# JaredWinkens/sdr-iq-visualizer

Hardware: AMD Instinct MI355X
Metric: complex64 IQ Msamples/s through windowed FFT+log-PSD, N=4096; % HBM3E peak (higher is better)
Workload: dtype f32

## Files before the change

### experiments/f4k_order/timeline.py

```python
import argparse
import ctypes
import json
import os
import sys

REPO = os.path.dirname(os.path.dirname(os.path.dirname(os.path.abspath(__file__))))
sys.path.insert(0, REPO)
import torch
import numpy as np
from bench import warm_up_by_time
from sdr_iq_visualizer_amd import _ffi
from sdr_iq_visualizer_amd.spectrum import SpectrumPlan

NFFT = 4096
TICK_NS = 10.0
BIN_MS = 0.5


def analyse(rec, n_frames):
    t = rec[:, 0].astype(np.uint64) | (rec[:, 1].astype(np.uint64) << np.uint64(32))
    assert (t > 0).all(), "frames without a record"
    assert np.array_equal(rec[:, 2], np.arange(n_frames, dtype=np.uint32)), "a record names another frame than its own"
    wg = rec[:, 3].astype(np.int64)
    grid = int(wg.max()) + 1
# ... 8 lines not shown
    cut = np.searchsorted(ms[order], np.arange(n_bins + 1) * BIN_MS, side="left")
    cut[-1] = n_frames
    for b in range(n_bins):
        hi = (b + 1) * BIN_MS
        idx = order[cut[b]:cut[b + 1]]
        if idx.size == 0:
            continue
        reached[wg[idx]] = frame[idx]
        active = (last_ms >= hi) & (reached >= 0)
        front = int(reached.max())
        lag = int(front - reached[active].min()) if active.any() else 0
        bins.append({"ms": round(b * BIN_MS, 2), "frames": int(idx.size), "span": int(frame[idx].max() - frame[idx].min()),
                     "lag_frames": lag, "lag_grids": round(lag / grid, 2)})
    return {"grid": grid, "launch_ms_by_records": round(float(ms.max()), 3), "bins": bins}


def main():
    ap = argparse.ArgumentParser()
    ap.add_argument("--out", required=True)
    ap.add_argument("--frames", type=int, default=1 << 20)
    ap.add_argument("--short", type=int, default=65536)
    ap.add_argument("--pairs", type=int, default=3)
    ap.add_argument("--orders", default="stride,ticket",
                    help="comma-separated SDRK_F4K_ORDER values, each optionally with :<SDRK_F4K_TICKET_FORM> (ticket:rot4)")
    a = ap.parse_args()
    lib = _ffi.lib()
    _ffi.require_device(0)
    set_tl = lib.sdrk_f4k_timeline
    set_tl.argtypes, set_tl.restype = [ctypes.c_void_p], ctypes.c_int
    os.environ["SDRK_F4K_PARTS"] = "1"
    d_in = ctypes.c_void_p()
    _ffi.check(lib.sdrk_dev_alloc(0, a.frames * NFFT * 8, ctypes.byref(d_in)))
    outs = []
    for _ in range(a.pairs):
        p = ctypes.c_void_p()
        _ffi.check(lib.sdrk_dev_alloc(0, a.frames * NFFT * 4, ctypes.byref(p)))
        outs.append(p)
    _ffi.check(lib.sdrk_synth_fill(0, 1234, 0, a.frames, NFFT, d_in, None))
    tl = torch.zeros((a.frames, 4), dtype=torch.int32, device="cuda")
    os.makedirs(os.path.dirname(os.path.abspath(a.out)), exist_ok=True)
    with open(a.out, "a") as out:
        for order in [o for o in a.orders.split(",") if o]:
            os.environ["SDRK_F4K_ORDER"] = order.split(":")[0]
            if ":" in order:
                os.environ["SDRK_F4K_TICKET_FORM"] = order.split(":")[1]
            else:
                os.environ.pop("SDRK_F4K_TICKET_FORM", None)
            with SpectrumPlan(NFFT, window="hann", device=0) as plan:
                warm_up_by_time(lambda: plan.exec_device_timed(d_in.value, a.frames, outs[0].value, 1))
                for i, p in enumerate(outs):
                    for n in (a.frames, a.short):
                        plan.exec_device_timed(d_in.value, n, p.value, 1)
                        tl.zero_()
                        torch.cuda.synchronize()
                        assert set_tl(tl.data_ptr()) == 0
                        ms = plan.exec_device_timed(d_in.value, n, p.value, 1)
                        assert set_tl(None) == 0
                        rec = tl[:n].cpu().numpy().view(np.uint32)
                        r = {"order": order, "pair": i, "frames": n, "launch_ms_by_events": round(float(ms), 4), **analyse(rec, n)}
                        out.write(json.dumps(r) + "\n")
                        out.flush()
                        print(f"== {order} pair {i} frames {n}: {r['launch_ms_by_events']} ms by events, "
                              f"{r['launch_ms_by_records']} ms first to last issue, grid {r['grid']}")
                        for b in r["bins"]:
                            print(f"   {b['ms']:5.2f} ms  frames {b['frames']:7d}  span {b['span']:8d}  lag {b['lag_frames']:8d} "
                                  f"frames = {b['lag_grids']:7.2f} grids", flush=True)
    for p in outs:
        lib.sdrk_dev_free(0, p)
    lib.sdrk_dev_free(0, d_in)

# ... 4 lines not shown
```

### sdr-iq-visualizer_amd/csrc/aux_kernels.hip

```cpp
#include "f4k_deal.h"
#include "kernels.h"
#include "synth_hash.h"

namespace sdrk {

__global__ __launch_bounds__(256) void synth_fill_kernel(uint32_t seed, uint64_t first_frame,
                                                         size_t n_frames, int nfft,
                                                         float4* __restrict__ out) {
    const size_t pairs_per_frame = (size_t)nfft / 2;
    const size_t total = n_frames * pairs_per_frame;
    for (size_t i = (size_t)blockIdx.x * blockDim.x + threadIdx.x; i < total;
         i += (size_t)gridDim.x * blockDim.x) {
        const size_t f = i / pairs_per_frame;
        const uint32_t n = (uint32_t)(i - f * pairs_per_frame) * 2u;
        const uint64_t F = first_frame + f;
        const uint32_t base = synth_frame_base(seed, F);
        int i0, q0, i1, q1;
        synth_codes(base, n, i0, q0);
        synth_codes(base, n + 1u, i1, q1);
        float4 v;
        v.x = (float)i0;
        v.y = (float)q0;
        v.z = (float)i1;
        v.w = (float)q1;
// ... 124 lines not shown
}

hipError_t launch_copy_1to1(const void* d_in, void* d_out, size_t bytes, int num_cus, int blocks_per_cu, hipStream_t stream) {
    const size_t n_vec = bytes / 16;
    if (n_vec == 0) return hipSuccess;
    size_t blocks = (n_vec + 1023) / 1024;
    if (blocks > (size_t)num_cus * blocks_per_cu) blocks = (size_t)num_cus * blocks_per_cu;
    hipLaunchKernelGGL(copy_1to1_kernel, dim3((unsigned)blocks), dim3(256), 0, stream, static_cast<const v4f*>(d_in),
                       static_cast<v4f*>(d_out), n_vec);
    return hipGetLastError();
}

template <class Deal>
__global__ __launch_bounds__(256) void stream_mix_dealt_kernel(const v4f* __restrict__ in, v4f* __restrict__ out, size_t n_frames,
                                                               const sdrk_host::F4kDealArgs da) {
    __shared__ unsigned deal_slot[F4K_DEAL_SLOTS];
    const int tid = threadIdx.x;
    Deal deal = Deal::make(da, n_frames, deal_slot, tid);
    deal.publish(tid);
    __syncthreads();
    deal.begin();
    while (deal.more()) {
        deal.top(tid);
        const size_t f = deal.frame();
        if (f < n_frames) {
            const v4f* x = in + f * 2048;
            v4f* o = out + f * 1024;
            v4f v[8];
#pragma unroll
            for (int j = 0; j < 8; ++j) v[j] = __builtin_nontemporal_load(&x[tid + 256 * j]);
#pragma unroll
            for (int j = 0; j < 4; ++j) __builtin_nontemporal_store(v[2 * j] + v[2 * j + 1], &o[tid + 256 * j]);
        }
        __syncthreads();
        deal.step();
    }
    deal.leave(tid);
}

template <class Deal>
__global__ __launch_bounds__(256) void copy_1to1_dealt_kernel(const v4f* __restrict__ in, v4f* __restrict__ out, size_t n_vec,
                                                              const sdrk_host::F4kDealArgs da) {
    __shared__ unsigned deal_slot[F4K_DEAL_SLOTS];
    const int tid = threadIdx.x;
    const size_t n_units = (n_vec + 1023) / 1024;
    Deal deal = Deal::make(da, n_units, deal_slot, tid);
    deal.publish(tid);
    __syncthreads();
    deal.begin();
    while (deal.more()) {
        deal.top(tid);
        const size_t u = deal.frame();
        if (u < n_units) {
            const size_t i = u * 1024 + tid;
            v4f v[4];
#pragma unroll
            for (int j = 0; j < 4; ++j)
                if (i + 256 * j < n_vec) v[j] = __builtin_nontemporal_load(&in[i + 256 * j]);
#pragma unroll
            for (int j = 0; j < 4; ++j)
                if (i + 256 * j < n_vec) __builtin_nontemporal_store(v[j], &out[i + 256 * j]);
        }
        __syncthreads();
        deal.step();
    }
    deal.leave(tid);
}

template <class Launch>
static hipError_t launch_dealt(sdrk_host::F4kProbeDeal& pd, size_t max_blocks, size_t n_units, Launch&& launch) {
    using namespace sdrk_host;
    if (!pd.d_heads || !f4k_ticket_takes(pd.choice.order, max_blocks, n_units, F4K_TICKET_DEFAULT)) return hipErrorNotSupported;
    const unsigned grid = f4k_ticket_grid(max_blocks, n_units);
    const F4kDealArgs da = {pd.d_heads, pd.bases, pd.choice.form, pd.choice.rot_heads};
    launch(grid, da, pd.choice.rot_heads != 0);
    const hipError_t e = hipGetLastError();
    if (e == hipSuccess && !pd.choice.rot_heads) f4k_ticket_advance(pd.choice.form, pd.bases, n_units, grid);
    return e;
}

hipError_t launch_stream_mix_dealt(const void* d_in, void* d_out, size_t n_frames4096, int num_cus, hipStream_t stream,
                                   sdrk_host::F4kProbeDeal& pd) {
    if (n_frames4096 == 0) return hipSuccess;
    const v4f* in = static_cast<const v4f*>(d_in);
    v4f* out = static_cast<v4f*>(d_out);
    const hipError_t e = launch_dealt(pd, (size_t)num_cus * 3, n_frames4096, [&](unsigned grid, const sdrk_host::F4kDealArgs& da, bool rot) {
        if (rot) hipLaunchKernelGGL(stream_mix_dealt_kernel<F4kRotDeal>, dim3(grid), dim3(256), 0, stream, in, out, n_frames4096, da);
        else hipLaunchKernelGGL(stream_mix_dealt_kernel<F4kTicketDeal>, dim3(grid), dim3(256), 0, stream, in, out, n_frames4096, da);
    });
    return e == hipErrorNotSupported ? launch_stream_mix(d_in, d_out, n_frames4096, num_cus, stream) : e;
}

hipError_t launch_copy_1to1_dealt(const void* d_in, void* d_out, size_t bytes, int num_cus, int blocks_per_cu, hipStream_t stream,
                                  sdrk_host::F4kProbeDeal& pd) {
    const size_t n_vec = bytes / 16;
    if (n_vec == 0) return hipSuccess;
    const v4f* in = static_cast<const v4f*>(d_in);
    v4f* out = static_cast<v4f*>(d_out);
    const hipError_t e = launch_dealt(pd, (size_t)num_cus * blocks_per_cu, (n_vec + 1023) / 1024,
                                      [&](unsigned grid, const sdrk_host::F4kDealArgs& da, bool rot) {
        if (rot) hipLaunchKernelGGL(copy_1to1_dealt_kernel<F4kRotDeal>, dim3(grid), dim3(256), 0, stream, in, out, n_vec, da);
        else hipLaunchKernelGGL(copy_1to1_dealt_kernel<F4kTicketDeal>, dim3(grid), dim3(256), 0, stream, in, out, n_vec, da);
    });
    return e == hipErrorNotSupported ? launch_copy_1to1(d_in, d_out, bytes, num_cus, blocks_per_cu, stream) : e;
}

hipError_t launch_power_mean(const void* d_spec, size_t n_frames, int nfft, float scale, float* d_out,
                             hipStream_t stream) {
    hipLaunchKernelGGL(power_mean_kernel, dim3((nfft + 255) / 256), dim3(256), 0, stream,
                       static_cast<const float2*>(d_spec), n_frames, nfft, scale, d_out);
    return hipGetLastError();
}

}
```

### sdr-iq-visualizer_amd/csrc/f4k_deal.h

```cpp
#pragma once
#include <hip/hip_runtime.h>

#include "f4k_rot.h"
#include "f4k_ticket.h"

namespace sdrk {

constexpr int F4K_DEAL_SLOTS = 4;

__device__ __forceinline__ unsigned f4k_deal_draw(unsigned* word, unsigned n) {
    return __hip_atomic_fetch_add(word, n, __ATOMIC_RELAXED, __HIP_MEMORY_SCOPE_AGENT);
}

struct F4kTicketDeal {
    sdrk_host::F4kTicketForm form;
    size_t n_frames, cur, nx, tn, in_ticket;
    unsigned* head;
    unsigned* slot;
    unsigned hx, base, depth, drawn, par;
    bool last_of_ticket;

    __device__ __forceinline__ F4kTicketDeal(unsigned* heads, const sdrk_host::F4kTicketBases& bases, sdrk_host::F4kTicketForm f,
                                             size_t n, unsigned* lds_slots, int tid)
        : form(f), n_frames(n), in_ticket(f.frames - 1), slot(lds_slots), hx(blockIdx.x & (f.heads - 1)),
          depth(sdrk_host::f4k_ticket_depth(f)), drawn(0), par(1), last_of_ticket(false) {
        head = heads + hx * sdrk_host::F4K_TICKET_HEAD_WORDS + __lane_id();
        base = bases.base[hx];
        if (tid == 0) drawn = f4k_deal_draw(head, depth);
    }
    static __device__ __forceinline__ F4kTicketDeal make(const sdrk_host::F4kDealArgs& a, size_t n, unsigned* lds_slots, int tid) {
        return F4kTicketDeal(a.heads, a.bases, a.form, n, lds_slots, tid);
    }
    __device__ __forceinline__ size_t first_of(unsigned head_value) const {
        return sdrk_host::f4k_ticket_first_frame(form, head_value - base, hx);
    }
    __device__ __forceinline__ void publish(int tid) {
        if (tid == 0) {
// ... 11 lines not shown
    __device__ __forceinline__ void top(int tid) {
        last_of_ticket = ((nx + 1) & in_ticket) == 0;
        if (last_of_ticket && tid == 0) {
            slot[par] = drawn;
            drawn = f4k_deal_draw(head, 1u);
        }
    }
    __device__ __forceinline__ size_t frame() const { return cur; }
    __device__ __forceinline__ size_t next() const { return nx; }
    __device__ __forceinline__ void step() {
        size_t after = nx + 1;
        if (last_of_ticket) {
            after = tn;
            tn = first_of(__builtin_amdgcn_readfirstlane(slot[par]));
            par ^= 1;
        }
        cur = nx;
        nx = after;
    }
    __device__ __forceinline__ void leave(int) {}
};

struct F4kRotDeal {
    sdrk_host::F4kRotDrawer dr;
    size_t n_frames;
    unsigned* lane_heads;
    unsigned* slot;
    unsigned drawn, d0, d1, h0, h1;
    unsigned cur, nx, par;

    __device__ __forceinline__ F4kRotDeal(unsigned* heads, unsigned n_heads, size_t n, unsigned* lds_slots, int tid)
        : dr(sdrk_host::f4k_rot_drawer(n_heads, blockIdx.x)), n_frames(n), lane_heads(heads + __lane_id()), slot(lds_slots),
          drawn(0), d0(0), d1(0), h0(0), h1(0), par(2) {
        if (tid == 0) {
            h0 = dr.head;
            d0 = f4k_deal_draw(word(h0), 1u);
            h1 = (h0 + 1) & (n_heads - 1);
            d1 = f4k_deal_draw(word(h1), 1u);
            dr.head = (h1 + 1) & (n_heads - 1);
            drawn = f4k_deal_draw(word(dr.head), 1u);
            dr.pending = true;
        }
    }
    static __device__ __forceinline__ F4kRotDeal make(const sdrk_host::F4kDealArgs& a, size_t n, unsigned* lds_slots, int tid) {
        return F4kRotDeal(a.heads, a.rot_heads, n, lds_slots, tid);
    }
// ... 18 lines not shown
            slot[par] = dr.pending ? sdrk_host::f4k_rot_take(dr, drawn, n_frames) : sdrk_host::F4K_ROT_NONE;
            if (sdrk_host::f4k_rot_advance(dr)) drawn = f4k_deal_draw(word(dr.head), 1u);
        }
    }
    __device__ __forceinline__ size_t frame() const { return cur; }
    __device__ __forceinline__ size_t next() const { return nx; }
    __device__ __forceinline__ void step() {
        const unsigned after = __builtin_amdgcn_readfirstlane(slot[par]);
        par ^= 1;
        cur = nx;
        nx = after;
    }
    __device__ __forceinline__ void leave(int tid) {
        if (tid == 0) {
            unsigned* const exits = lane_heads + sdrk_host::F4K_ROT_EXIT_WORD;
            if (f4k_deal_draw(exits, 1u) == gridDim.x - 1) {
                for (unsigned x = 0; x < dr.heads; ++x) __hip_atomic_store(word(x), 0u, __ATOMIC_RELAXED, __HIP_MEMORY_SCOPE_AGENT);
                __hip_atomic_store(exits, 0u, __ATOMIC_RELAXED, __HIP_MEMORY_SCOPE_AGENT);
            }
        }
    }
};

}
```

### sdr-iq-visualizer_amd/csrc/f4k_rot.h

```cpp
#pragma once
#include <cstddef>
#include <cstdint>
#include <cstdio>

#include "f4k_ticket.h"

namespace sdrk_host {

constexpr unsigned F4K_ROT_AHEAD = 3;
constexpr unsigned F4K_ROT_EXIT_WORD = F4K_TICKET_MAX_HEADS * F4K_TICKET_HEAD_WORDS;
constexpr unsigned F4K_ROT_WORDS = (F4K_TICKET_MAX_HEADS + 1) * F4K_TICKET_HEAD_WORDS;
constexpr uint32_t F4K_ROT_NONE = 0xFFFFFFFFu;

constexpr bool f4k_rot_heads_ok(unsigned heads) { return heads == 2 || heads == 4 || heads == 8; }

constexpr uint32_t f4k_rot_frame(unsigned heads, uint32_t ticket, unsigned head) { return ticket * heads + head; }

constexpr unsigned f4k_rot_next_head(unsigned heads, unsigned live, unsigned last) {
    const unsigned twice = live | (live << heads);
    return (last + 1 + (unsigned)__builtin_ctz(twice >> (last + 1))) & (heads - 1);
}

struct F4kRotDrawer {
    unsigned heads;
// ... 3 lines not shown
};
constexpr F4kRotDrawer f4k_rot_drawer(unsigned heads, unsigned workgroup) {
    return F4kRotDrawer{heads, (1u << heads) - 1u, workgroup & (heads - 1), false};
}
constexpr uint32_t f4k_rot_take(F4kRotDrawer& d, uint32_t ticket, size_t n_frames) {
    const uint32_t fr = f4k_rot_frame(d.heads, ticket, d.head);
    if (fr >= n_frames) d.live &= ~(1u << d.head);
    return fr;
}
constexpr bool f4k_rot_advance(F4kRotDrawer& d) {
    d.pending = d.live != 0;
    if (d.pending) d.head = f4k_rot_next_head(d.heads, d.live, d.head);
    return d.pending;
}

inline unsigned f4k_rot_parse(const char* s) {
    if (!s || s[0] != 'r' || s[1] != 'o' || s[2] != 't' || s[3] == 0 || s[4] != 0) return 0;
    const unsigned h = (unsigned)(s[3] - '0');
    return f4k_rot_heads_ok(h) ? h : 0;
}

constexpr unsigned F4K_ROT_DEFAULT_HEADS = 4;

struct F4kChoice {
    int order = F4K_ORDER_AUTO;
    F4kTicketForm form = F4K_TICKET_FORM;
    unsigned rot_heads = F4K_ROT_DEFAULT_HEADS;
};
inline F4kChoice f4k_choice(const char* order_env, const char* form_env) {
    F4kChoice c;
    if (order_env) c.order = order_env[0] == 't' ? F4K_ORDER_TICKET : (order_env[0] == 's' ? F4K_ORDER_STRIDE : F4K_ORDER_AUTO);
    if (form_env) {
        F4kTicketForm f = {0, 0};
        if (const unsigned rot = f4k_rot_parse(form_env)) c.rot_heads = rot;
        else if (sscanf(form_env, "%ux%u", &f.heads, &f.frames) == 2 && f4k_ticket_form_ok(f)) { c.form = f; c.rot_heads = 0; }
    }
    return c;
}

struct F4kDealArgs {
    unsigned* heads;
    F4kTicketBases bases;
    F4kTicketForm form;
    unsigned rot_heads;
};

struct F4kProbeDeal {
    F4kChoice choice;
    unsigned* d_heads = nullptr;
    F4kTicketBases bases = {};
};

}
// ... 1 lines not shown
```

### sdr-iq-visualizer_amd/csrc/fft4096.hip

```cpp
#include "f4k_deal.h"
#include "fft4096_core.h"

namespace sdrk {

#ifdef SDRK_F4K_TIMELINE
__device__ uint4* f4k_timeline_buf = nullptr;
#define F4K_TIMELINE_LOAD() uint4* const f4k_tl = f4k_timeline_buf
#define F4K_TIMELINE_MARK(fr)                                                                                   \
    do {                                                                                                        \
        if (f4k_tl && tid == 0 && (fr) < n_frames) {                                                            \
            const unsigned long long f4k_t = wall_clock64();                                                    \
            f4k_tl[fr] = make_uint4((unsigned)f4k_t, (unsigned)(f4k_t >> 32), (unsigned)(fr), blockIdx.x);      \
        }                                                                                                       \
    } while (0)
#else
#define F4K_TIMELINE_LOAD() (void)0
#define F4K_TIMELINE_MARK(fr) (void)0
#endif

template <bool HAS_WINDOW, int EPILOGUE>
__global__ __launch_bounds__(F4K_THREADS, F4K_WAVES) void fft4096_kernel(
    const float2* __restrict__ iq, size_t frame_stride, void* __restrict__ out_raw,
    size_t n_frames, const float* __restrict__ window, const float2* __restrict__ tw4096,
    float eps, int shift) {
// ... 149 lines not shown
        In::issue(x, iq + fr * frame_stride, tid);
    };
    In::word nxt[16];
    deal.begin();
    issue(nxt, deal.frame());
    while (deal.more()) {
        deal.top(tid);
        const size_t cur = deal.frame();
        if (cur < n_frames) {
            In::to_owners(nxt, lds, tid);
            cf v[16];
#pragma unroll
            for (int j = 0; j < 16; ++j) v[j] = In::widen(nxt[j]);
            issue(nxt, deal.next());
            f4k_windowed_transform<HAS_WINDOW>(v, lds, tw256, tw1, lds_win, A, tid);
            deal.step();
            f4k_store_row<EPILOGUE>(v, frame_rsrc(static_cast<char*>(out_raw) + cur * (size_t)(F4K_N * OUT_ELEM), F4K_N * OUT_ELEM),
                                    voff_out, xor_k2, eps);
        } else {
            issue(nxt, deal.next());
            __syncthreads();
            deal.step();
        }
    }
    deal.leave(tid);
}

unsigned f4k_max_blocks(int num_cus) { return f4k_grid(num_cus, F4K_WAVES, (size_t)-1); }

hipError_t launch_fft4096(const LaunchArgs& a) {
    if (a.n_frames == 0) return hipSuccess;
    dim3 g(f4k_grid(a.num_cus, F4K_WAVES, a.n_frames)), b(F4K_THREADS);
    const float2* iq = static_cast<const float2*>(a.d_iq);
    const float2* tw = static_cast<const float2*>(a.d_twiddle);
#define SDRK_LAUNCH(W, E)                                                                            \
    hipLaunchKernelGGL((fft4096_kernel<W, E>), g, b, 0, a.stream, iq, a.frame_stride, a.d_out,           \
                       a.n_frames, a.d_window, tw, a.eps, a.shift)
    if (a.epilogue == EPI_LOGPSD) {
        if (a.d_window) SDRK_LAUNCH(true, EPI_LOGPSD); else SDRK_LAUNCH(false, EPI_LOGPSD);
    } else {
        if (a.d_window) SDRK_LAUNCH(true, EPI_COMPLEX); else SDRK_LAUNCH(false, EPI_COMPLEX);
    }
#undef SDRK_LAUNCH
    return hipGetLastError();
}

// ... 16 lines not shown
    return hipGetLastError();
}

hipError_t launch_fft4096_rot(const LaunchArgs& a, unsigned* d_heads, unsigned n_heads, unsigned grid) {
    if (a.n_frames == 0) return hipSuccess;
    if (!d_heads || grid == 0 || grid % sdrk_host::F4K_TICKET_MAX_HEADS || !sdrk_host::f4k_rot_heads_ok(n_heads) ||
        a.n_frames > sdrk_host::F4K_TICKET_MAX_FRAMES)
        return hipErrorInvalidValue;
    dim3 g(grid), b(F4K_THREADS);
    const float2* iq = static_cast<const float2*>(a.d_iq);
    const float2* tw = static_cast<const float2*>(a.d_twiddle);
#define SDRK_LAUNCH(W, E)                                                                            \
    hipLaunchKernelGGL((fft4096_rot_kernel<W, E>), g, b, 0, a.stream, iq, a.frame_stride, a.d_out,       \
                       a.n_frames, a.d_window, tw, a.eps, a.shift, d_heads, n_heads)
    if (a.epilogue == EPI_LOGPSD) {
        if (a.d_window) SDRK_LAUNCH(true, EPI_LOGPSD); else SDRK_LAUNCH(false, EPI_LOGPSD);
    } else {
        if (a.d_window) SDRK_LAUNCH(true, EPI_COMPLEX); else SDRK_LAUNCH(false, EPI_COMPLEX);
    }
#undef SDRK_LAUNCH
    return hipGetLastError();
}

}

#ifdef SDRK_F4K_TIMELINE
extern "C" int sdrk_f4k_timeline(void* d_records) {
    uint4* p = static_cast<uint4*>(d_records);
    return (int)hipMemcpyToSymbol(HIP_SYMBOL(sdrk::f4k_timeline_buf), &p, sizeof p);
}
#endif
```

### sdr-iq-visualizer_amd/csrc/fft4096_core.h

```cpp
#pragma once
#include "cplx.h"
#include "kernels.h"

namespace sdrk {

constexpr int F4K_N = 4096;
constexpr int F4K_THREADS = 256;
#ifndef F4K_WAVES
#define F4K_WAVES 3
#endif
constexpr int F4K_XCH_ELEMS = 4112;
constexpr int F4K_TW_ELEMS = 512;
#ifndef F4K_NT
#define F4K_NT 2
#endif
constexpr int f4k_lds_elems(bool lds_window) { return F4K_XCH_ELEMS + F4K_TW_ELEMS + (lds_window ? F4K_N / 2 : 0); }

typedef unsigned v2u __attribute__((ext_vector_type(2)));

__device__ __forceinline__ __amdgpu_buffer_rsrc_t frame_rsrc(const void* base, unsigned bytes) {
    return __builtin_amdgcn_make_buffer_rsrc(const_cast<void*>(base), 0, (int)bytes, 0x00020000);
}


// ... 22 lines not shown
    const int lo = tid & 15, hi = tid >> 4;
    tw256[tid] = tw4096[(16 * lo * hi) & (F4K_N - 1)];
    tw1[tid] = tw4096[tid];
}

__device__ __forceinline__ void pow_tree(cf w1, cf (&w)[16]) {
    w[1] = w1;
    w[2] = cmul(w1, w1);
    w[3] = cmul(w[2], w1);
    w[4] = cmul(w[2], w[2]);
    w[5] = cmul(w[4], w1);
    w[6] = cmul(w[4], w[2]);
    w[7] = cmul(w[4], w[3]);
    w[8] = cmul(w[4], w[4]);
    w[9] = cmul(w[8], w1);
    w[10] = cmul(w[8], w[2]);
    w[11] = cmul(w[8], w[3]);
    w[12] = cmul(w[8], w[4]);
    w[13] = cmul(w[8], w[5]);
    w[14] = cmul(w[8], w[6]);
    w[15] = cmul(w[8], w[7]);
}

template <bool WIN = false>
__device__ __forceinline__ void f4k_transform(cf (&v)[16], float2* __restrict__ lds,
                                              const float2* __restrict__ tw256,
                                              const float2* __restrict__ tw1, const F4kAddr& A,
                                              int tid, const float* __restrict__ win = nullptr) {
    radix16<WIN>(v, win);
    {
        const float2 t1 = tw1[tid];
        cf w[16];
        pow_tree(cf{t1.x, t1.y}, w);
#pragma unroll
        for (int k = 1; k < 16; ++k) v[rev16(k)] = cmul(v[rev16(k)], w[k]);
    }
    __syncthreads();
#pragma unroll
    for (int k = 0; k < 16; ++k)
        lds[((k & 1) ? A.x1w_odd : A.x1w_even) + 256 * k] = make_float2(v[rev16(k)].x, v[rev16(k)].y);
    __syncthreads();
#pragma unroll
    for (int j = 0; j < 16; ++j) {
        float2 t = lds[((j & 1) ? A.x1r_odd : A.x1r_even) + 16 * j];
        v[j] = cf{t.x, t.y};
    }
    radix16(v);
#pragma unroll
    for (int k = 1; k < 16; ++k) {
        float2 w = tw256[16 * k + A.lo];
        v[rev16(k)] = cmul(v[rev16(k)], cf{w.x, w.y});
    }
    __syncthreads();
#pragma unroll
    for (int k = 0; k < 16; ++k) lds[A.x2w + 16 * k] = make_float2(v[rev16(k)].x, v[rev16(k)].y);
    __syncthreads();
#pragma unroll
    for (int j = 0; j < 16; ++j) {
        float2 t = lds[tid + 257 * j];
        v[j] = cf{t.x, t.y};
// ... 2 lines not shown
}


inline unsigned f4k_grid(int num_cus, int wg_per_cu, size_t work_items) {
    const size_t max_blocks = (size_t)num_cus * wg_per_cu;
    return (unsigned)(work_items < max_blocks ? work_items : max_blocks);
}

struct F4kInC64 {
    typedef v2u word;
    typedef float2 sample;
    static __device__ __forceinline__ void issue(word (&x)[16], const sample* frame, int tid) {
        __amdgpu_buffer_rsrc_t r = frame_rsrc(frame, F4K_N * 8);
#pragma unroll
        for (int j = 0; j < 16; ++j) x[j] = __builtin_amdgcn_raw_buffer_load_b64(r, tid * 8, j * 2048, F4K_NT);
    }
    static __device__ __forceinline__ void to_owners(word (&)[16], float2*, int) {}
    static __device__ __forceinline__ cf widen(word w) {
        v2f t = __builtin_bit_cast(v2f, w);
        return cf{t.x, t.y};
    }
};

template <bool HAS_WINDOW>
__device__ __forceinline__ void f4k_windowed_transform(cf (&v)[16], float2* __restrict__ lds, const float2* __restrict__ tw256,
                                                       const float2* __restrict__ tw1, const float* __restrict__ lds_win,
                                                       const F4kAddr& A, int tid) {
    if (HAS_WINDOW) {
        float win[16];
#pragma unroll
        for (int j = 0; j < 16; ++j) win[j] = lds_win[tid + 256 * j];
        f4k_transform<true>(v, lds, tw256, tw1, A, tid, win);
    } else {
        f4k_transform(v, lds, tw256, tw1, A, tid);
    }
}

template <int EPILOGUE>
__device__ __forceinline__ void f4k_store_row(const cf (&v)[16], __amdgpu_buffer_rsrc_t w, int voff, int xor_k2, float eps) {
    if (EPILOGUE == EPI_LOGPSD) {
#pragma unroll
        for (int k2 = 0; k2 < 16; ++k2) {
            cf z = v[rev16(k2)];
            float db = logpsd_db(z.x, z.y, eps);
            __builtin_amdgcn_raw_buffer_store_b32(__builtin_bit_cast(unsigned, db), w, voff, (k2 ^ xor_k2) * 1024, F4K_NT);
        }
    } else {
#pragma unroll
        for (int k2 = 0; k2 < 16; ++k2) {
            cf z = v[rev16(k2)];
            v2f o = {z.x, z.y};
            __builtin_amdgcn_raw_buffer_store_b64(__builtin_bit_cast(v2u, o), w, voff, (k2 ^ xor_k2) * 2048, 0);
        }
    }
}

}
// ... 1 lines not shown
```

### sdr-iq-visualizer_amd/csrc/kernels.h

```cpp
#pragma once
#include <hip/hip_runtime.h>
#include <stddef.h>
#include <stdint.h>

#include <atomic>

#include "f4k_ticket.h"
#include "f4k_rot.h"

#ifdef SDRK_PHASE_MARKS
#define SDRK_PHASE(name) asm volatile("; SDRK_PHASE " name ::: "memory")
#else
#define SDRK_PHASE(name) do { } while (0)
#endif

namespace sdrk {

enum Epilogue : int {
    EPI_LOGPSD = 0,
    EPI_COMPLEX = 1,
    EPI_BLU_MUL = 2,
    EPI_BLU_POST_LOG = 3,
    EPI_BLU_POST_C64 = 4,
};
// ... 34 lines not shown
__device__ __forceinline__ float logpsd_db_fast(float p) {
    return __builtin_amdgcn_logf(p) * 3.01029995663981195213f;
}

#endif

inline hipError_t ensure_dynamic_lds(const void* kernel, size_t lds_bytes, std::atomic<uint64_t>& mask) {
    if (lds_bytes <= 64 * 1024) return hipSuccess;
    int dev = 0;
    hipError_t e = hipGetDevice(&dev);
    if (e != hipSuccess) return e;
    const uint64_t bit = (dev >= 0 && dev < 64) ? (uint64_t)1 << dev : 0;
    if (bit && (mask.load(std::memory_order_acquire) & bit)) return hipSuccess;
    e = hipFuncSetAttribute(kernel, hipFuncAttributeMaxDynamicSharedMemorySize, (int)lds_bytes);
    if (e == hipSuccess && bit) mask.fetch_or(bit, std::memory_order_release);
    return e;
}

hipError_t launch_fft4096(const LaunchArgs& a);
unsigned f4k_max_blocks(int num_cus);
hipError_t launch_fft4096_ticket(const LaunchArgs& a, unsigned* d_heads, const sdrk_host::F4kTicketBases& bases,
                                 sdrk_host::F4kTicketForm form, unsigned grid);
hipError_t launch_fft4096_rot(const LaunchArgs& a, unsigned* d_heads, unsigned n_heads, unsigned grid);
hipError_t launch_fft_small(const LaunchArgs& a);
bool fft_lds_supports(int nfft);
hipError_t launch_fft_lds(const LaunchArgs& a);
bool fft_tiled2_split(int nfft, int* log2a, int* log2m);
hipError_t launch_fft_tiled2(const LaunchArgs& a);
bool fft_tiled2_has_mip(int nfft, int epilogue);
hipError_t launch_synth_fill(uint32_t seed, uint64_t first_frame, size_t n_frames, int nfft,
                             void* d_iq, hipStream_t stream);

size_t fused64k_ring_bytes();
size_t fused64k_ctrl_words();
unsigned fused64k_sets(int num_cus);
hipError_t launch_fused64k(const LaunchArgs& a, void* d_ring, unsigned* d_ctrl);
bool blu_fused_supports(int M);
hipError_t launch_blu_fused(const void* d_iq, size_t frame_stride, size_t n_frames, int N, int M, const float* d_window,
                            const void* d_chirp, const void* d_bspec, const void* d_twM, float eps, int shift,
                            int epilogue, void* d_out, int num_cus, hipStream_t s);
hipError_t launch_blu_pre(const void* d_iq, size_t frame_stride, size_t n_frames, int N, int M, const float* d_window,
                          const void* d_chirp, void* d_a, int num_cus, hipStream_t s, bool compact = false);
hipError_t launch_blu_mul(const void* d_A, const void* d_B, size_t n_frames, int M, void* d_out, int num_cus,
                          hipStream_t s);
hipError_t launch_blu_post(const void* d_Y, const void* d_chirp, size_t n_frames, int N, int M, float eps, int shift,
                           int epilogue, void* d_out, int num_cus, hipStream_t s);
// ... 25 lines not shown
```

### sdr-iq-visualizer_amd/csrc/plan_internal.h

```cpp
#pragma once
#include <hip/hip_runtime.h>

#include <cstddef>
#include <cstdint>
#include <map>
#include <mutex>
#include <utility>
#include <vector>

#include "../../include/sdrk.h"
#include "kernels.h"

namespace sdrk_host {
constexpr int HOST_SLOTS = 3;
struct ChunkOut {
    enum Rows {
        None,
        Pooled,
        Direct,
        Kernel,
        Planes,
    } rows = None;
    void* user = nullptr;
    size_t bytes = 0;
// ... 72 lines not shown
    int precision = 32;
    double eps64 = 0.0;
    double* d_window64 = nullptr;
    double* d_tw64 = nullptr;
    void* d_scratch64 = nullptr;
    sdrk_host::Staging ci16;
    sdrk_host::Staging integ;
    float* d_pfb_h = nullptr;
    int pfb_taps = 0;
    int pfb_assign = 0;
    sdrk_host::Staging pfb;
    float2* d_fir_h = nullptr;
    int fir_taps = 0;
    int fir_assign = 0;
    float2* d_beam_h = nullptr;
    int beam_channels = 0;
    int beam_taps = 0;
    int f4k_order = sdrk_host::F4K_ORDER_AUTO;
    sdrk_host::F4kTicketForm f4k_form = sdrk_host::F4K_TICKET_FORM;
    unsigned* d_f4k_heads = nullptr;
    sdrk_host::F4kTicketBases f4k_bases = {};
    unsigned f4k_rot_heads = sdrk_host::F4K_ROT_DEFAULT_HEADS;
    unsigned* d_f4k_rot = nullptr;
    hipEvent_t f4k_ev = nullptr;
    hipStream_t f4k_last = nullptr;
    bool f4k_recorded = false;
    size_t f4k_parts = 0;
};

namespace sdrk_host {

constexpr size_t SMALL_IN_BYTES = 256 << 10;
constexpr size_t HOST_CHUNK_BYTES = 16 << 20;
constexpr size_t ZERO_COPY_MAX_BYTES = 32 << 20;
constexpr unsigned FUSED_MAILBOX = 64;
constexpr size_t FUSED_AUTO_MIN_FRAMES = 512;

int fail(int status, const char* fmt, ...) __attribute__((format(printf, 2, 3)));

#define HIP_TRY(expr)                                                                                                   \
    do {                                                                                                                \
        hipError_t e__ = (expr);                                                                                        \
        if (e__ != hipSuccess)                                                                                          \
            return ::sdrk_host::fail(e__ == hipErrorOutOfMemory ? SDRK_ERR_NOMEM : SDRK_ERR_HIP,                        \
                                     "%s failed: %s (%s:%d)", #expr, hipGetErrorString(e__), __FILE__, __LINE__);       \
    } while (0)
// ... 197 lines not shown
```

### sdr-iq-visualizer_amd/csrc/sdrk_plan.hip

```cpp
#include "../../include/sdrk.h"

#include <hip/hip_runtime.h>

#include <cmath>
#include <cstdio>
#include <cstdlib>
#include <cstring>
#include <dlfcn.h>
#include <mutex>
#include <new>
#include <vector>

#include "f4k_split.h"
#include "kernels.h"
#include "plan_internal.h"

using namespace sdrk_host;

namespace sdrk_host {

struct EpiArgs {
    const float2* tab = nullptr;
    int n_out = 0;
    float eps = 0.0f;
// ... 129 lines not shown
            if (st != SDRK_OK) return st;
            e = sdrk::launch_blu_mul(p->d_blu_b, p->d_blu_bspec, nf, M, p->d_blu_a, p->num_cus, stream);
            if (e != hipSuccess) break;
            st = plan_launch(p->blu_inner, p->d_blu_a, nf, (size_t)M, p->d_blu_b, sdrk::EPI_COMPLEX, stream);
            if (st != SDRK_OK) return st;
            e = sdrk::launch_blu_post(p->d_blu_b, p->d_blu_chirp, nf, N, M, p->eps, p->shift, epilogue,
                                      static_cast<char*>(d_out) + f0 * (size_t)N * out_elem, p->num_cus, stream);
            if (e != hipSuccess) break;
        }
    } else if (p->nfft == 4096) {
        const size_t max_blocks = sdrk::f4k_max_blocks(p->num_cus);
        const bool ticket = p->d_f4k_heads && f4k_ticket_takes(p->f4k_order, max_blocks, n_frames, F4K_TICKET_DEFAULT);
        size_t parts = p->f4k_parts ? p->f4k_parts : (ticket ? f4k_ticket_parts(n_frames) : f4k_split_parts(n_frames));
        if (p->f4k_parts && parts > n_frames) parts = n_frames ? n_frames : 1;
        const size_t per = (n_frames + parts - 1) / parts;
        const size_t out_elem = epilogue == sdrk::EPI_LOGPSD ? sizeof(float) : sizeof(float2);
        if (ticket && p->f4k_recorded && p->f4k_last != stream) e = hipStreamWaitEvent(stream, p->f4k_ev, 0);
        for (size_t f0 = 0; f0 < n_frames && e == hipSuccess; f0 += per) {
            a.d_iq = static_cast<const float2*>(d_iq) + f0 * frame_stride;
            a.d_out = static_cast<char*>(d_out) + f0 * (size_t)4096 * out_elem;
            a.n_frames = n_frames - f0 < per ? n_frames - f0 : per;
            if (ticket) {
                const unsigned grid = f4k_ticket_grid(max_blocks, a.n_frames);
                if (p->f4k_rot_heads) {
                    e = sdrk::launch_fft4096_rot(a, p->d_f4k_rot, p->f4k_rot_heads, grid);
                } else {
                    e = sdrk::launch_fft4096_ticket(a, p->d_f4k_heads, p->f4k_bases, p->f4k_form, grid);
                    if (e == hipSuccess) f4k_ticket_advance(p->f4k_form, p->f4k_bases, a.n_frames, grid);
                }
            } else {
                e = sdrk::launch_fft4096(a);
            }
        }
        if (ticket && e == hipSuccess) {
            e = hipEventRecord(p->f4k_ev, stream);
            p->f4k_last = stream;
            p->f4k_recorded = true;
        }
    } else if (sdrk::fft_lds_supports(p->nfft))
        e = sdrk::launch_fft_lds(a);
    else if (p->nfft < 4096)
        e = sdrk::launch_fft_small(a);
    else if (takes_fused(p, call_frames) && !d_mip && epilogue <= sdrk::EPI_COMPLEX) {
        FusedGate& gate = fused_gate(p->device);
        std::lock_guard<std::mutex> lk(gate.mu);
        if (gate.ev && gate.last_stream != stream && gate.recorded) e = hipStreamWaitEvent(stream, gate.ev, 0);
        if (e == hipSuccess) e = sdrk::launch_fused64k(a, p->d_fused_ring, p->d_fused_ctrl);
// ... 168 lines not shown
            const double ang = M_PI * (double)r / (double)nfft;
            c[n] = make_float2((float)std::cos(ang), (float)std::sin(ang));
            b[n] = c[n];
            if (n) b[M - n] = c[n];
        }
        PLAN_TRY(hipMalloc((void**)&p->d_blu_chirp, sizeof(float2) * nfft));
        PLAN_TRY(hipMemcpy(p->d_blu_chirp, c.data(), sizeof(float2) * nfft, hipMemcpyHostToDevice));
        PLAN_TRY(hipMalloc((void**)&p->d_blu_a, (one_kernel ? 1 : frames) * (size_t)M * sizeof(float2)));
        if (!one_kernel) PLAN_TRY(hipMalloc((void**)&p->d_blu_b, frames * (size_t)M * sizeof(float2)));
        PLAN_TRY(hipMalloc((void**)&p->d_blu_bspec, (size_t)M * sizeof(float2)));
        PLAN_TRY(hipMemcpy(p->d_blu_a, b.data(), sizeof(float2) * M, hipMemcpyHostToDevice));
        st2 = plan_launch(p->blu_inner, p->d_blu_a, 1, (size_t)M, p->d_blu_bspec, sdrk::EPI_COMPLEX, p->stream);
        if (st2 != SDRK_OK) { sdrk_plan_destroy(p); return st2; }
        PLAN_TRY(hipStreamSynchronize(p->stream));
        *out = p;
        return SDRK_OK;
    }
    if (nfft <= 16384) {
        std::vector<float2> t(nfft);
        for (int m = 0; m < nfft; ++m) t[m] = twiddle(m, nfft);
        PLAN_TRY(hipMalloc((void**)&p->d_twiddle, sizeof(float2) * nfft));
        PLAN_TRY(hipMemcpy(p->d_twiddle, t.data(), sizeof(float2) * nfft, hipMemcpyHostToDevice));
        if (nfft == 4096) {
            const F4kChoice choice = f4k_choice(getenv("SDRK_F4K_ORDER"), getenv("SDRK_F4K_TICKET_FORM"));
            p->f4k_order = choice.order;
            p->f4k_form = choice.form;
            p->f4k_rot_heads = choice.rot_heads;
            if (const char* env = getenv("SDRK_F4K_PARTS")) {
                long v = atol(env);
                if (v >= 1 && v <= 4096) p->f4k_parts = (size_t)v;
            }
            PLAN_TRY(hipMalloc((void**)&p->d_f4k_rot, F4K_ROT_WORDS * sizeof(uint32_t)));
            const std::vector<uint32_t> rot0(F4K_ROT_WORDS, 0u);
            PLAN_TRY(hipMemcpy(p->d_f4k_rot, rot0.data(), rot0.size() * sizeof(uint32_t), hipMemcpyHostToDevice));
            std::vector<uint32_t> h(F4K_TICKET_MAX_HEADS * F4K_TICKET_HEAD_WORDS, 0u);
            for (unsigned x = 0; x < F4K_TICKET_MAX_HEADS; ++x) h[x * F4K_TICKET_HEAD_WORDS] = p->f4k_bases.base[x] = 0xFFFFFE00u;
            PLAN_TRY(hipMalloc((void**)&p->d_f4k_heads, h.size() * sizeof(uint32_t)));
            PLAN_TRY(hipMemcpy(p->d_f4k_heads, h.data(), h.size() * sizeof(uint32_t), hipMemcpyHostToDevice));
            PLAN_TRY(hipEventCreateWithFlags(&p->f4k_ev, hipEventDisableTiming));
        }
    } else {
        size_t scratch_mb = 192;
        if (const char* env = getenv("SDRK_SCRATCH_MB")) {
            long v = atol(env);
            if (v >= 1 && v <= 65536) scratch_mb = (size_t)v;
        }
        size_t frames = (scratch_mb << 20) / ((size_t)nfft * sizeof(float2));
        if (frames < 1) frames = 1;
        if (frames > max_batch) frames = max_batch;
        p->scratch_frames = frames;
// ... 164 lines not shown
```

### sdr-iq-visualizer_amd/csrc/sdrk_probes.hip

```cpp
#include "../../include/sdrk.h"

#include <hip/hip_runtime.h>

#include <algorithm>
#include <chrono>
#include <cstring>
#include <vector>

#include "kernels.h"
#include "plan_internal.h"

using namespace sdrk_host;

namespace sdrk_host {
namespace {

thread_local int g_probe_status = SDRK_OK;
hipError_t probe_launch_result(int st) {
    if (st == SDRK_OK) return hipSuccess;
    g_probe_status = st;
    return hipErrorUnknown;
}
int probe_fail(hipError_t e, const char* what) {
    if (e == hipErrorUnknown && g_probe_status != SDRK_OK) {
// ... 60 lines not shown
    hipEvent_t e0 = nullptr, e1 = nullptr;
    HIP_TRY(hipStreamCreateWithFlags(&s, hipStreamNonBlocking));
    hipError_t e = hipEventCreate(&e0);
    if (e == hipSuccess) e = hipEventCreate(&e1);
    for (int i = -2; i < launches && e == hipSuccess; ++i) {
        if (i >= 0) e = hipEventRecord(e0, s);
        if (e == hipSuccess) e = launch(prop.multiProcessorCount, s);
        if (i >= 0 && e == hipSuccess) e = hipEventRecord(e1, s);
        if (i >= 0 && e == hipSuccess) e = hipEventSynchronize(e1);
        if (i >= 0 && e == hipSuccess) e = hipEventElapsedTime(&each_ms[i], e0, e1);
    }
    (void)hipStreamSynchronize(s);
    if (e0) (void)hipEventDestroy(e0);
    if (e1) (void)hipEventDestroy(e1);
    (void)hipStreamDestroy(s);
    if (e != hipSuccess) return fail(SDRK_ERR_HIP, "%s failed: %s", what, hipGetErrorString(e));
    return SDRK_OK;
}

struct ProbeHeads {
    F4kProbeDeal deal;
    int status = SDRK_OK;
    explicit ProbeHeads(int device) {
        deal.choice = f4k_choice(getenv("SDRK_F4K_ORDER"), getenv("SDRK_F4K_TICKET_FORM"));
        if (deal.choice.order == F4K_ORDER_STRIDE) return;
        status = check_device(device);
        if (status != SDRK_OK) return;
        const std::vector<uint32_t> zero(F4K_ROT_WORDS, 0u);
        hipError_t e = hipSetDevice(device);
        if (e == hipSuccess) e = hipMalloc((void**)&deal.d_heads, zero.size() * sizeof(uint32_t));
        if (e == hipSuccess) e = hipMemcpy(deal.d_heads, zero.data(), zero.size() * sizeof(uint32_t), hipMemcpyHostToDevice);
        if (e != hipSuccess) status = fail(SDRK_ERR_HIP, "probe heads: %s", hipGetErrorString(e));
    }
    ~ProbeHeads() {
        if (deal.d_heads) (void)hipFree(deal.d_heads);
    }
    ProbeHeads(const ProbeHeads&) = delete;
    ProbeHeads& operator=(const ProbeHeads&) = delete;
};

}

int tune_staging(sdrk_plan* p) {
    const size_t nfft = (size_t)p->nfft;
    if (p->blu_inner || p->max_batch * nfft * sizeof(float2) <= 2 * HOST_CHUNK_BYTES) return SDRK_OK;
    size_t per = HOST_CHUNK_BYTES / (nfft * sizeof(float2));
    if (per < 1) per = 1;
// ... 313 lines not shown
```

Before: 538,800.

## Add two-ahead rotating-head frame dealer with deferred draw for FFT4096

Adds a new rotating-head work dealer (F4kRotDeal2) that publishes the next frame index at the top of each iteration and issues the atomic draw for the following frame after the compute body. This keeps the atomic's latency off the critical path between frames. A new fft4096_rot2 kernel and dealt copy/mix probe kernels use this dealer, and it becomes the default via SDRK_F4K_ROT_AHEAD. The cost is an extra barrier per iteration, double-buffered LDS slots, and more complex dealing logic.

After: 557,300, median of 6. +3.4%, better.

```diff
diff --git a/experiments/f4k_order/timeline.py b/experiments/f4k_order/timeline.py
--- a/experiments/f4k_order/timeline.py
+++ b/experiments/f4k_order/timeline.py
@@ -54,7 +54,8 @@
     ap.add_argument("--short", type=int, default=65536)
     ap.add_argument("--pairs", type=int, default=3)
     ap.add_argument("--orders", default="stride,ticket",
-                    help="comma-separated SDRK_F4K_ORDER values, each optionally with :<SDRK_F4K_TICKET_FORM> (ticket:rot4)")
+                    help="comma-separated SDRK_F4K_ORDER values, each optionally with :<SDRK_F4K_TICKET_FORM> (ticket:rot4) and, for a "
+                         "rot form, @<SDRK_F4K_ROT_AHEAD> (ticket:rot4@3)")
     a = ap.parse_args()
     lib = _ffi.lib()
     _ffi.require_device(0)
@@ -74,10 +75,12 @@
     with open(a.out, "a") as out:
         for order in [o for o in a.orders.split(",") if o]:
             os.environ["SDRK_F4K_ORDER"] = order.split(":")[0]
-            if ":" in order:
-                os.environ["SDRK_F4K_TICKET_FORM"] = order.split(":")[1]
-            else:
-                os.environ.pop("SDRK_F4K_TICKET_FORM", None)
+            form, _, ahead = order.partition(":")[2].partition("@")
+            for var, value in (("SDRK_F4K_TICKET_FORM", form), ("SDRK_F4K_ROT_AHEAD", ahead)):
+                if value:
+                    os.environ[var] = value
+                else:
+                    os.environ.pop(var, None)
             with SpectrumPlan(NFFT, window="hann", device=0) as plan:
                 warm_up_by_time(lambda: plan.exec_device_timed(d_in.value, a.frames, outs[0].value, 1))
                 for i, p in enumerate(outs):
diff --git a/sdr-iq-visualizer_amd/csrc/aux_kernels.hip b/sdr-iq-visualizer_amd/csrc/aux_kernels.hip
--- a/sdr-iq-visualizer_amd/csrc/aux_kernels.hip
+++ b/sdr-iq-visualizer_amd/csrc/aux_kernels.hip
@@ -170,6 +170,10 @@
     deal.begin();
     while (deal.more()) {
         deal.top(tid);
+        if constexpr (Deal::TWO_AHEAD) {
+            __syncthreads();
+            deal.read();
+        }
         const size_t f = deal.frame();
         if (f < n_frames) {
             const v4f* x = in + f * 2048;
@@ -180,7 +184,8 @@
 #pragma unroll
             for (int j = 0; j < 4; ++j) __builtin_nontemporal_store(v[2 * j] + v[2 * j + 1], &o[tid + 256 * j]);
         }
-        __syncthreads();
+        if constexpr (Deal::TWO_AHEAD) deal.tail(tid);
+        else __syncthreads();
         deal.step();
     }
     deal.leave(tid);
@@ -198,6 +203,10 @@
     deal.begin();
     while (deal.more()) {
         deal.top(tid);
+        if constexpr (Deal::TWO_AHEAD) {
+            __syncthreads();
+            deal.read();
+        }
         const size_t u = deal.frame();
         if (u < n_units) {
             const size_t i = u * 1024 + tid;
@@ -209,7 +218,8 @@
             for (int j = 0; j < 4; ++j)
                 if (i + 256 * j < n_vec) __builtin_nontemporal_store(v[j], &out[i + 256 * j]);
         }
-        __syncthreads();
+        if constexpr (Deal::TWO_AHEAD) deal.tail(tid);
+        else __syncthreads();
         deal.step();
     }
     deal.leave(tid);
@@ -221,7 +231,7 @@
     if (!pd.d_heads || !f4k_ticket_takes(pd.choice.order, max_blocks, n_units, F4K_TICKET_DEFAULT)) return hipErrorNotSupported;
     const unsigned grid = f4k_ticket_grid(max_blocks, n_units);
     const F4kDealArgs da = {pd.d_heads, pd.bases, pd.choice.form, pd.choice.rot_heads};
-    launch(grid, da, pd.choice.rot_heads != 0);
+    launch(grid, da, !pd.choice.rot_heads ? 0 : (pd.choice.rot_ahead == F4K_AHEAD_2TOP ? 2 : 1));
     const hipError_t e = hipGetLastError();
     if (e == hipSuccess && !pd.choice.rot_heads) f4k_ticket_advance(pd.choice.form, pd.bases, n_units, grid);
     return e;
@@ -232,8 +242,9 @@
     if (n_frames4096 == 0) return hipSuccess;
     const v4f* in = static_cast<const v4f*>(d_in);
     v4f* out = static_cast<v4f*>(d_out);
-    const hipError_t e = launch_dealt(pd, (size_t)num_cus * 3, n_frames4096, [&](unsigned grid, const sdrk_host::F4kDealArgs& da, bool rot) {
-        if (rot) hipLaunchKernelGGL(stream_mix_dealt_kernel<F4kRotDeal>, dim3(grid), dim3(256), 0, stream, in, out, n_frames4096, da);
+    const hipError_t e = launch_dealt(pd, (size_t)num_cus * 3, n_frames4096, [&](unsigned grid, const sdrk_host::F4kDealArgs& da, int rot) {
+        if (rot == 2) hipLaunchKernelGGL(stream_mix_dealt_kernel<F4kRotDeal2>, dim3(grid), dim3(256), 0, stream, in, out, n_frames4096, da);
+        else if (rot) hipLaunchKernelGGL(stream_mix_dealt_kernel<F4kRotDeal>, dim3(grid), dim3(256), 0, stream, in, out, n_frames4096, da);
         else hipLaunchKernelGGL(stream_mix_dealt_kernel<F4kTicketDeal>, dim3(grid), dim3(256), 0, stream, in, out, n_frames4096, da);
     });
     return e == hipErrorNotSupported ? launch_stream_mix(d_in, d_out, n_frames4096, num_cus, stream) : e;
@@ -246,8 +257,9 @@
     const v4f* in = static_cast<const v4f*>(d_in);
     v4f* out = static_cast<v4f*>(d_out);
     const hipError_t e = launch_dealt(pd, (size_t)num_cus * blocks_per_cu, (n_vec + 1023) / 1024,
-                                      [&](unsigned grid, const sdrk_host::F4kDealArgs& da, bool rot) {
-        if (rot) hipLaunchKernelGGL(copy_1to1_dealt_kernel<F4kRotDeal>, dim3(grid), dim3(256), 0, stream, in, out, n_vec, da);
+                                      [&](unsigned grid, const sdrk_host::F4kDealArgs& da, int rot) {
+        if (rot == 2) hipLaunchKernelGGL(copy_1to1_dealt_kernel<F4kRotDeal2>, dim3(grid), dim3(256), 0, stream, in, out, n_vec, da);
+        else if (rot) hipLaunchKernelGGL(copy_1to1_dealt_kernel<F4kRotDeal>, dim3(grid), dim3(256), 0, stream, in, out, n_vec, da);
         else hipLaunchKernelGGL(copy_1to1_dealt_kernel<F4kTicketDeal>, dim3(grid), dim3(256), 0, stream, in, out, n_vec, da);
     });
     return e == hipErrorNotSupported ? launch_copy_1to1(d_in, d_out, bytes, num_cus, blocks_per_cu, stream) : e;
diff --git a/sdr-iq-visualizer_amd/csrc/f4k_deal.h b/sdr-iq-visualizer_amd/csrc/f4k_deal.h
--- a/sdr-iq-visualizer_amd/csrc/f4k_deal.h
+++ b/sdr-iq-visualizer_amd/csrc/f4k_deal.h
@@ -13,6 +13,7 @@
 }
 
 struct F4kTicketDeal {
+    static constexpr bool TWO_AHEAD = false;
     sdrk_host::F4kTicketForm form;
     size_t n_frames, cur, nx, tn, in_ticket;
     unsigned* head;
@@ -70,6 +71,7 @@
 };
 
 struct F4kRotDeal {
+    static constexpr bool TWO_AHEAD = false;
     sdrk_host::F4kRotDrawer dr;
     size_t n_frames;
     unsigned* lane_heads;
@@ -134,4 +136,62 @@
     }
 };
 
+struct F4kRotDeal2 {
+    static constexpr bool TWO_AHEAD = true;
+    sdrk_host::F4kRotDrawer dr;
+    size_t n_frames;
+    unsigned* lane_heads;
+    unsigned* slot;
+    unsigned drawn, d0, h0;
+    unsigned cur, nx, par;
+
+    __device__ __forceinline__ F4kRotDeal2(unsigned* heads, unsigned n_heads, size_t n, unsigned* lds_slots, int tid)
+        : dr(sdrk_host::f4k_rot_drawer(n_heads, blockIdx.x)), n_frames(n), lane_heads(heads + __lane_id()), slot(lds_slots),
+          drawn(0), d0(0), h0(0), cur(0), nx(sdrk_host::F4K_ROT_NONE), par(2) {
+        if (tid == 0) {
+            h0 = dr.head;
+            d0 = f4k_deal_draw(word(h0), 1u);
+            dr.head = (h0 + 1) & (n_heads - 1);
+            drawn = f4k_deal_draw(word(dr.head), 1u);
+            dr.pending = true;
+        }
+    }
+    static __device__ __forceinline__ F4kRotDeal2 make(const sdrk_host::F4kDealArgs& a, size_t n, unsigned* lds_slots, int tid) {
+        return F4kRotDeal2(a.heads, a.rot_heads, n, lds_slots, tid);
+    }
+    __device__ __forceinline__ unsigned* word(unsigned head) const { return lane_heads + head * sdrk_host::F4K_TICKET_HEAD_WORDS; }
+    __device__ __forceinline__ void publish(int tid) {
+        if (tid == 0) {
+            const unsigned h1 = dr.head;
+            dr.head = h0;
+            slot[0] = sdrk_host::f4k_rot_take(dr, d0, n_frames);
+            dr.head = h1;
+        }
+    }
+    __device__ __forceinline__ void begin() { cur = __builtin_amdgcn_readfirstlane(slot[0]); }
+    __device__ __forceinline__ bool more() const { return cur != sdrk_host::F4K_ROT_NONE; }
+    __device__ __forceinline__ void top(int tid) {
+        if (tid == 0) slot[par] = dr.pending ? sdrk_host::f4k_rot_take(dr, drawn, n_frames) : sdrk_host::F4K_ROT_NONE;
+    }
+    __device__ __forceinline__ void read() {
+        nx = __builtin_amdgcn_readfirstlane(slot[par]);
+        par ^= 1;
+    }
+    __device__ __forceinline__ size_t frame() const { return cur; }
+    __device__ __forceinline__ size_t next() const { return nx; }
+    __device__ __forceinline__ void tail(int tid) {
+        if (tid == 0 && sdrk_host::f4k_rot_advance(dr)) drawn = f4k_deal_draw(word(dr.head), 1u);
+    }
+    __device__ __forceinline__ void step() { cur = nx; }
+    __device__ __forceinline__ void leave(int tid) {
+        if (tid == 0) {
+            unsigned* const exits = lane_heads + sdrk_host::F4K_ROT_EXIT_WORD;
+            if (f4k_deal_draw(exits, 1u) == gridDim.x - 1) {
+                for (unsigned x = 0; x < dr.heads; ++x) __hip_atomic_store(word(x), 0u, __ATOMIC_RELAXED, __HIP_MEMORY_SCOPE_AGENT);
+                __hip_atomic_store(exits, 0u, __ATOMIC_RELAXED, __HIP_MEMORY_SCOPE_AGENT);
+            }
+        }
+    }
+};
+
 }
diff --git a/sdr-iq-visualizer_amd/csrc/f4k_rot.h b/sdr-iq-visualizer_amd/csrc/f4k_rot.h
--- a/sdr-iq-visualizer_amd/csrc/f4k_rot.h
+++ b/sdr-iq-visualizer_amd/csrc/f4k_rot.h
@@ -49,13 +49,24 @@
 
 constexpr unsigned F4K_ROT_DEFAULT_HEADS = 4;
 
+enum { F4K_AHEAD_3 = 3, F4K_AHEAD_2TOP = 2 };
+constexpr int F4K_ROT_DEFAULT_AHEAD = F4K_AHEAD_2TOP;
+
 struct F4kChoice {
     int order = F4K_ORDER_AUTO;
     F4kTicketForm form = F4K_TICKET_FORM;
     unsigned rot_heads = F4K_ROT_DEFAULT_HEADS;
+    int rot_ahead = F4K_ROT_DEFAULT_AHEAD;
 };
-inline F4kChoice f4k_choice(const char* order_env, const char* form_env) {
+inline int f4k_rot_ahead_parse(const char* s) {
+    if (!s) return -1;
+    if (s[0] == '3' && s[1] == 0) return F4K_AHEAD_3;
+    if (s[0] == '2' && s[1] == 't' && s[2] == 'o' && s[3] == 'p' && s[4] == 0) return F4K_AHEAD_2TOP;
+    return -1;
+}
+inline F4kChoice f4k_choice(const char* order_env, const char* form_env, const char* ahead_env = nullptr) {
     F4kChoice c;
+    if (const int ahead = f4k_rot_ahead_parse(ahead_env); ahead >= 0) c.rot_ahead = ahead;
     if (order_env) c.order = order_env[0] == 't' ? F4K_ORDER_TICKET : (order_env[0] == 's' ? F4K_ORDER_STRIDE : F4K_ORDER_AUTO);
     if (form_env) {
         F4kTicketForm f = {0, 0};
diff --git a/sdr-iq-visualizer_amd/csrc/fft4096.hip b/sdr-iq-visualizer_amd/csrc/fft4096.hip
--- a/sdr-iq-visualizer_amd/csrc/fft4096.hip
+++ b/sdr-iq-visualizer_amd/csrc/fft4096.hip
@@ -195,6 +195,65 @@
             __syncthreads();
             deal.step();
         }
+    }
+    deal.leave(tid);
+}
+
+template <bool HAS_WINDOW, int EPILOGUE>
+__global__ __launch_bounds__(F4K_THREADS, F4K_WAVES) void fft4096_rot2_kernel(
+    const float2* __restrict__ iq, size_t frame_stride, void* __restrict__ out_raw,
+    size_t n_frames, const float* __restrict__ window, const float2* __restrict__ tw4096,
+    float eps, int shift, unsigned* __restrict__ heads, const unsigned n_heads) {
+    typedef F4kInC64 In;
+    __shared__ float2 lds[f4k_lds_elems(HAS_WINDOW)];
+    __shared__ unsigned deal_slot[F4K_DEAL_SLOTS];
+    float2* __restrict__ tw256 = lds + F4K_XCH_ELEMS;
+    float2* __restrict__ tw1 = tw256 + 256;
+    float* __restrict__ lds_win = reinterpret_cast<float*>(tw1 + 256);
+
+    const int tid = threadIdx.x;
+    F4kRotDeal2 deal(heads, n_heads, n_frames, deal_slot, tid);
+    F4kAddr A = f4k_addr(tid);
+    f4k_init_tables(tw256, tw1, tw4096, tid);
+    if (HAS_WINDOW) {
+#pragma unroll
+        for (int j = 0; j < 16; ++j) lds_win[tid + 256 * j] = window[tid + 256 * j];
+    }
+    deal.publish(tid);
+    __syncthreads();
+
+    const int xor_k2 = shift ? 8 : 0;
+    constexpr int OUT_ELEM = (EPILOGUE == EPI_LOGPSD ? 4 : 8);
+    const int voff_out = tid * OUT_ELEM;
+    F4K_TIMELINE_LOAD();
+
+    auto issue = [&](In::word (&x)[16], size_t fr) {
+        F4K_TIMELINE_MARK(fr);
+        if (fr >= n_frames) fr = 0;
+        In::issue(x, iq + fr * frame_stride, tid);
+    };
+    In::word nxt[16];
+    deal.begin();
+    issue(nxt, deal.frame());
+    while (deal.more()) {
+        deal.top(tid);
+        __syncthreads();
+        deal.read();
+        const size_t cur = deal.frame();
+        if (cur < n_frames) {
+            In::to_owners(nxt, lds, tid);
+            cf v[16];
+#pragma unroll
+            for (int j = 0; j < 16; ++j) v[j] = In::widen(nxt[j]);
+            issue(nxt, deal.next());
+            f4k_windowed_transform<HAS_WINDOW, false>(v, lds, tw256, tw1, lds_win, A, tid);
+            f4k_store_row<EPILOGUE>(v, frame_rsrc(static_cast<char*>(out_raw) + cur * (size_t)(F4K_N * OUT_ELEM), F4K_N * OUT_ELEM),
+                                    voff_out, xor_k2, eps);
+        } else {
+            issue(nxt, deal.next());
+        }
+        deal.tail(tid);
+        deal.step();
     }
     deal.leave(tid);
 }
@@ -257,6 +316,26 @@
     return hipGetLastError();
 }
 
+hipError_t launch_fft4096_rot2(const LaunchArgs& a, unsigned* d_heads, unsigned n_heads, unsigned grid) {
+    if (a.n_frames == 0) return hipSuccess;
+    if (!d_heads || grid == 0 || grid % sdrk_host::F4K_TICKET_MAX_HEADS || !sdrk_host::f4k_rot_heads_ok(n_heads) ||
+        a.n_frames > sdrk_host::F4K_TICKET_MAX_FRAMES)
+        return hipErrorInvalidValue;
+    dim3 g(grid), b(F4K_THREADS);
+    const float2* iq = static_cast<const float2*>(a.d_iq);
+    const float2* tw = static_cast<const float2*>(a.d_twiddle);
+#define SDRK_LAUNCH(W, E)                                                                            \
+    hipLaunchKernelGGL((fft4096_rot2_kernel<W, E>), g, b, 0, a.stream, iq, a.frame_stride, a.d_out,      \
+                       a.n_frames, a.d_window, tw, a.eps, a.shift, d_heads, n_heads)
+    if (a.epilogue == EPI_LOGPSD) {
+        if (a.d_window) SDRK_LAUNCH(true, EPI_LOGPSD); else SDRK_LAUNCH(false, EPI_LOGPSD);
+    } else {
+        if (a.d_window) SDRK_LAUNCH(true, EPI_COMPLEX); else SDRK_LAUNCH(false, EPI_COMPLEX);
+    }
+#undef SDRK_LAUNCH
+    return hipGetLastError();
+}
+
 }
 
 #ifdef SDRK_F4K_TIMELINE
diff --git a/sdr-iq-visualizer_amd/csrc/fft4096_core.h b/sdr-iq-visualizer_amd/csrc/fft4096_core.h
--- a/sdr-iq-visualizer_amd/csrc/fft4096_core.h
+++ b/sdr-iq-visualizer_amd/csrc/fft4096_core.h
@@ -68,7 +68,7 @@
     w[15] = cmul(w[8], w[7]);
 }
 
-template <bool WIN = false>
+template <bool WIN = false, bool ENTRY_BARRIER = true>
 __device__ __forceinline__ void f4k_transform(cf (&v)[16], float2* __restrict__ lds,
                                               const float2* __restrict__ tw256,
                                               const float2* __restrict__ tw1, const F4kAddr& A,
@@ -81,7 +81,7 @@
 #pragma unroll
         for (int k = 1; k < 16; ++k) v[rev16(k)] = cmul(v[rev16(k)], w[k]);
     }
-    __syncthreads();
+    if (ENTRY_BARRIER) __syncthreads();
 #pragma unroll
     for (int k = 0; k < 16; ++k)
         lds[((k & 1) ? A.x1w_odd : A.x1w_even) + 256 * k] = make_float2(v[rev16(k)].x, v[rev16(k)].y);
@@ -130,7 +130,7 @@
     }
 };
 
-template <bool HAS_WINDOW>
+template <bool HAS_WINDOW, bool ENTRY_BARRIER = true>
 __device__ __forceinline__ void f4k_windowed_transform(cf (&v)[16], float2* __restrict__ lds, const float2* __restrict__ tw256,
                                                        const float2* __restrict__ tw1, const float* __restrict__ lds_win,
                                                        const F4kAddr& A, int tid) {
@@ -138,9 +138,9 @@
         float win[16];
 #pragma unroll
         for (int j = 0; j < 16; ++j) win[j] = lds_win[tid + 256 * j];
-        f4k_transform<true>(v, lds, tw256, tw1, A, tid, win);
+        f4k_transform<true, ENTRY_BARRIER>(v, lds, tw256, tw1, A, tid, win);
     } else {
-        f4k_transform(v, lds, tw256, tw1, A, tid);
+        f4k_transform<false, ENTRY_BARRIER>(v, lds, tw256, tw1, A, tid);
     }
 }
 
diff --git a/sdr-iq-visualizer_amd/csrc/kernels.h b/sdr-iq-visualizer_amd/csrc/kernels.h
--- a/sdr-iq-visualizer_amd/csrc/kernels.h
+++ b/sdr-iq-visualizer_amd/csrc/kernels.h
@@ -80,6 +80,7 @@
 hipError_t launch_fft4096_ticket(const LaunchArgs& a, unsigned* d_heads, const sdrk_host::F4kTicketBases& bases,
                                  sdrk_host::F4kTicketForm form, unsigned grid);
 hipError_t launch_fft4096_rot(const LaunchArgs& a, unsigned* d_heads, unsigned n_heads, unsigned grid);
+hipError_t launch_fft4096_rot2(const LaunchArgs& a, unsigned* d_heads, unsigned n_heads, unsigned grid);
 hipError_t launch_fft_small(const LaunchArgs& a);
 bool fft_lds_supports(int nfft);
 hipError_t launch_fft_lds(const LaunchArgs& a);
diff --git a/sdr-iq-visualizer_amd/csrc/plan_internal.h b/sdr-iq-visualizer_amd/csrc/plan_internal.h
--- a/sdr-iq-visualizer_amd/csrc/plan_internal.h
+++ b/sdr-iq-visualizer_amd/csrc/plan_internal.h
@@ -118,6 +118,7 @@
     sdrk_host::F4kTicketBases f4k_bases = {};
     unsigned f4k_rot_heads = sdrk_host::F4K_ROT_DEFAULT_HEADS;
     unsigned* d_f4k_rot = nullptr;
+    int f4k_rot_ahead = sdrk_host::F4K_ROT_DEFAULT_AHEAD;
     hipEvent_t f4k_ev = nullptr;
     hipStream_t f4k_last = nullptr;
     bool f4k_recorded = false;
diff --git a/sdr-iq-visualizer_amd/csrc/sdrk_plan.hip b/sdr-iq-visualizer_amd/csrc/sdrk_plan.hip
--- a/sdr-iq-visualizer_amd/csrc/sdrk_plan.hip
+++ b/sdr-iq-visualizer_amd/csrc/sdrk_plan.hip
@@ -175,7 +175,9 @@
             a.n_frames = n_frames - f0 < per ? n_frames - f0 : per;
             if (ticket) {
                 const unsigned grid = f4k_ticket_grid(max_blocks, a.n_frames);
-                if (p->f4k_rot_heads) {
+                if (p->f4k_rot_heads && p->f4k_rot_ahead == F4K_AHEAD_2TOP) {
+                    e = sdrk::launch_fft4096_rot2(a, p->d_f4k_rot, p->f4k_rot_heads, grid);
+                } else if (p->f4k_rot_heads) {
                     e = sdrk::launch_fft4096_rot(a, p->d_f4k_rot, p->f4k_rot_heads, grid);
                 } else {
                     e = sdrk::launch_fft4096_ticket(a, p->d_f4k_heads, p->f4k_bases, p->f4k_form, grid);
@@ -390,10 +392,11 @@
         PLAN_TRY(hipMalloc((void**)&p->d_twiddle, sizeof(float2) * nfft));
         PLAN_TRY(hipMemcpy(p->d_twiddle, t.data(), sizeof(float2) * nfft, hipMemcpyHostToDevice));
         if (nfft == 4096) {
-            const F4kChoice choice = f4k_choice(getenv("SDRK_F4K_ORDER"), getenv("SDRK_F4K_TICKET_FORM"));
+            const F4kChoice choice = f4k_choice(getenv("SDRK_F4K_ORDER"), getenv("SDRK_F4K_TICKET_FORM"), getenv("SDRK_F4K_ROT_AHEAD"));
             p->f4k_order = choice.order;
             p->f4k_form = choice.form;
             p->f4k_rot_heads = choice.rot_heads;
+            p->f4k_rot_ahead = choice.rot_ahead;
             if (const char* env = getenv("SDRK_F4K_PARTS")) {
                 long v = atol(env);
                 if (v >= 1 && v <= 4096) p->f4k_parts = (size_t)v;
diff --git a/sdr-iq-visualizer_amd/csrc/sdrk_probes.hip b/sdr-iq-visualizer_amd/csrc/sdrk_probes.hip
--- a/sdr-iq-visualizer_amd/csrc/sdrk_probes.hip
+++ b/sdr-iq-visualizer_amd/csrc/sdrk_probes.hip
@@ -106,7 +106,7 @@
     F4kProbeDeal deal;
     int status = SDRK_OK;
     explicit ProbeHeads(int device) {
-        deal.choice = f4k_choice(getenv("SDRK_F4K_ORDER"), getenv("SDRK_F4K_TICKET_FORM"));
+        deal.choice = f4k_choice(getenv("SDRK_F4K_ORDER"), getenv("SDRK_F4K_TICKET_FORM"), getenv("SDRK_F4K_ROT_AHEAD"));
         if (deal.choice.order == F4K_ORDER_STRIDE) return;
         status = check_device(device);
         if (status != SDRK_OK) return;
```
